# grunwaldlab/krisp

Measured on AMD Instinct MI355X. Metric: k-mers/s sorted+intersected at k=28, higher is better.
Workload: dtype u64

## Files before the change

include/krisp_hip.h:

```cpp
#ifndef KRISP_HIP_H
#define KRISP_HIP_H

#include <stddef.h>
#include <stdint.h>

#ifdef __cplusplus
extern "C" {
#endif

typedef struct kr_ctx kr_ctx;

typedef struct { uint64_t prefix, in_mask, out_mask; } kr_cand;

typedef struct { uint64_t key; uint32_t genome; uint32_t count; } kr_record;

enum {
    KR_OK = 0,
    KR_ERR_HIP = -1,
    KR_ERR_PARAM = -2,
    KR_ERR_CAPACITY = -3,
    KR_ERR_STATE = -4,
    KR_ERR_KEY = -5,
    KR_ERR_HOST = -6
};
// ... 208 lines not shown

int64_t kr_render_records(const kr_record* recs, size_t n, int L, int D, int R, const uint32_t* label_of,
                          size_t n_genomes, const char* const* label_text, size_t n_labels, const uint8_t* label_in,
                          int dot, char** csv, size_t* csv_len, char** align, size_t* align_len);
int64_t kr_render_windows(const uint8_t* rows, size_t n, int L, int D, int R, const uint32_t* cand, const uint32_t* genome,
                          const uint32_t* label_of, size_t n_genomes, const char* const* label_text, size_t n_labels,
                          const uint8_t* label_in, int dot, int rna, char** csv, size_t* csv_len, char** align,
                          size_t* align_len);
void    kr_text_free(void* p);

enum { KR_OPT_SLICE_BASES = 1,
       KR_OPT_GENERIC_INTERSECT = 2,
       KR_OPT_ISECT_FORMAT = 3,
       KR_OPT_ABLATE = 4,
       KR_OPT_WIDE_SLOTS = 5,
       KR_OPT_PLACE_TRIES = 7,
       KR_OPT_ISECT_KERNEL = 8,
       KR_OPT_LANES = 9,
       KR_OPT_LAZY_ORDER = 10,
       KR_OPT_COARSE_REST = 11,
       KR_OPT_COARSE_POOL = 12,
       KR_OPT_JOIN2 = 13,
       KR_OPT_COARSE_ONE_STRAND = 14,
       KR_OPT_WIDE_ORDERED = 6 };
int     kr_set_option(kr_ctx*, int option, int64_t value);

int     kr_sync(kr_ctx*);
int     kr_timer_begin(kr_ctx*);
double  kr_timer_end_ms(kr_ctx*);
int     kr_stage_enable(kr_ctx*, int on);
int     kr_stage_select(kr_ctx*, unsigned stage_mask);
int     kr_stage_reset(kr_ctx*);
double  kr_stage_ms(kr_ctx*, int stage);
int64_t kr_stage_launches(kr_ctx*, int stage);

int64_t kr_debug_fetch(kr_ctx*, int genome_id, int what, void* out, size_t cap_bytes);
int64_t kr_debug_inversions(kr_ctx*, int genome_id);
double  kr_debug_localsort(kr_ctx*, int genome_id, int reps, int mode);
double  kr_debug_intersect(kr_ctx*, const int* genome_ids, int n, const uint8_t* is_ingroup, int reps, int mode);
double  kr_debug_copy_gbps(kr_ctx*, size_t bytes, int reps);
const char* kr_debug_copy_which(kr_ctx*);
int     kr_build_experiments(void);
int     kr_debug_lazy(kr_ctx*, int64_t* out8);
int     kr_debug_isect(kr_ctx*, int64_t* out8);
int     kr_debug_scan(kr_ctx*, int64_t* out8);
int     kr_debug_place(kr_ctx*, double* out8);
int     kr_debug_coarse_pool(kr_ctx*, double* out8);
int     kr_debug_coarse_strand(kr_ctx*, int64_t* out8);
int     kr_debug_comm(kr_ctx*, int64_t* out8);
int     kr_debug_comm_probe(kr_ctx*, size_t bytes, int reps, double* out3);
int64_t kr_debug_cands_selfexchange(kr_ctx*, int apply_filter);
int     kr_debug_comm_hang(kr_ctx*);
int64_t kr_debug_budget_left(kr_ctx*);
int     kr_debug_budget_set(kr_ctx*, int64_t left);
int     kr_debug_info(kr_ctx*, int64_t* out8);

#ifdef __cplusplus
}
#endif
#endif
```

krisp_amd/_native.py:

```python
import ctypes
import os

import numpy as np

HERE = os.path.dirname(os.path.abspath(__file__))
LIB_PATH = os.environ.get("KRISP_HIP_LIB") or os.path.join(HERE, "libkrisp_hip.so")

CAND = np.dtype([("prefix", "<u8"), ("in_mask", "<u8"), ("out_mask", "<u8")])
RECORD = np.dtype([("key", "<u8"), ("genome", "<u4"), ("count", "<u4")])
WIDE_HIT = np.dtype([("cand", "<u4"), ("genome", "<u4"), ("pos", "<u4"), ("strand", "<u4")])
LOC_HIT = np.dtype([("group", "<u4"), ("strand", "<u4"), ("pos", "<u8")])
NEAR_HIT = np.dtype([("target", "<u4"), ("strand", "u1"), ("mismatches", "u1"), ("flank_mismatches", "u1"), ("pad", "u1"),
                     ("pos", "<u8")])
PRODUCT_SITE = np.dtype([("pos", "<u8"), ("entry", "<u4"), ("mismatches", "u1"), ("end_mismatches", "u1"),
                         ("pad", "<u2")])
PRODUCT_HIT = np.dtype([("pos", "<u8"), ("length", "<u4"), ("pair", "<u4"), ("strand", "u1"), ("left_mm", "u1"),
                        ("right_mm", "u1"), ("left_end_mm", "u1"), ("right_end_mm", "u1"), ("pad", "u1", (3,))])
MULTIPLEX_HIT = np.dtype([("pos", "<u8"), ("length", "<u4"), ("fwd", "<u2"), ("rev", "<u2"), ("fwd_mm", "u1"), ("rev_mm", "u1"),
                          ("fwd_end_mm", "u1"), ("rev_end_mm", "u1"), ("pad", "u1", (4,))])
DESIGN_RECORD = np.dtype([("found", "<u4"), ("product_size", "<u4"), ("pair_penalty", "<u4"), ("left_start", "<u2"),
                          ("left_len", "<u2"), ("right_start", "<u2"), ("right_len", "<u2"), ("left_tm", "<i4"), ("right_tm", "<i4"),
                          ("left_gc", "<u2"), ("right_gc", "<u2"), ("left_penalty", "<u4"), ("right_penalty", "<u4"),
                          ("left_self_any", "<i4"), ("left_self_end", "<i4"), ("right_self_any", "<i4"),
                          ("right_self_end", "<i4"), ("pair_any", "<i4"), ("pair_end", "<i4")])
# ... 3 lines not shown
GUIDE_RECORD = np.dtype([("found", "<u4"), ("strand", "<u4"), ("start", "<u4"), ("min_mismatches", "<u4"),
                         ("sum_mismatches", "<u4"), ("gc", "<u4"), ("candidates", "<u4"), ("pad", "<u4")])
GUIDE_HIT_RAW = np.dtype([("guide", "<u4"), ("strand", "u1"), ("mismatches", "u1"), ("pam", "u1"), ("pad", "u1"), ("pos", "<u8"),
                          ("columns", "<u8")])
ASSAY_HIT_RAW = np.dtype([("pos", "<u8"), ("length", "<u4"), ("pair", "<u4"), ("strand", "u1"), ("left_mm", "u1"), ("right_mm", "u1"),
                          ("left_end_mm", "u1"), ("right_end_mm", "u1"), ("hit_strand", "u1"), ("hit_mismatches", "u1"),
                          ("hit_pam", "u1"), ("hit_pos", "<u8"), ("columns", "<u8"), ("guide", "<u4"), ("hit", "<u4")])
GUIDE_BULGE_HIT_RAW = np.dtype([("guide", "<u4"), ("strand", "u1"), ("mismatches", "u1"), ("pam", "u1"), ("bulge", "i1"),
                                ("pos", "<u8"), ("columns", "<u8"), ("bulge_column", "<u4"), ("length", "<u4")])
WIDE_DICT_LEFT, WIDE_DICT_RIGHT, WIDE_GROUPS, WIDE_HITS, WIDE_COUNTS, WIDE_SLOT_BITS, WIDE_NGROUPS, WIDE_BATCH_USED, WIDE_LOCATED, WIDE_KEYS_LISTED = 0, 1, 2, 3, 4, 5, 6, 7, 8, 9
WIDE_MAX_K = 1024
WIDE_MAX_FLANK = 256
COMM_ID_BYTES = 128

SOFT_MAP, SOFT_OMIT = 0, 1
OPT_SLICE_BASES, OPT_GENERIC_INTERSECT, OPT_ISECT_FORMAT, OPT_ABLATE, OPT_WIDE_SLOTS, OPT_WIDE_ORDERED, OPT_PLACE_TRIES = 1, 2, 3, 4, 5, 6, 7
OPT_ISECT_KERNEL = 8
OPT_LANES = 9
OPT_LAZY_ORDER = 10
OPT_COARSE_REST = 11
OPT_COARSE_POOL = 12
OPT_JOIN2 = 13
OPT_COARSE_ONE_STRAND = 14
ERR_KEY, ERR_HOST = -5, -6
STRANDS_BOTH, STRANDS_FORWARD, STRANDS_CANONICAL = 0, 1, 2
STAGES = ["pack", "hist8", "reduce8", "scatter1", "hist2", "scan2", "scatter2", "chunks", "localsort",
          "fallback", "intersect", "compact", "collect", "merge", "locate"]
STAGE_KERNELS = {"pack": "k_pack", "hist8": "k_hist8 (wide path: k_hist8w, slices: k_hist8k)", "reduce8": "k_reduce8a+k_reduce8b",
                 "scatter1": "k_scatter1p (wide path: k_scatter1w, slices: k_scatter1kp)",
                 "hist2": "k_hist16 (or k_hist2)", "scan2": "k_hist16_off (or k_scan2)", "scatter2": "k_scatter2",
                 "chunks": "k_chunk_table", "localsort": "k_localsort2",
                 "fallback": "k_seg_merge", "intersect": "k_intersect3 (+ k_intersect for oversized items)",
                 "compact": "k_scan+k_publish_reset+k_gather_items",
                 "collect": "k_collect_count+k_tile_sums+k_scan+k_tile_apply+k_publish+k_collect_emit",
                 "merge": "k_cands_flag+k_scan+k_cands_compact", "locate": "k_wide_locate"}

_c = ctypes
_P = _c.c_void_p
SYMBOLS = [
    ("kr_create", _P, [_c.c_int, _c.c_size_t]),
    ("kr_destroy", None, [_P]),
    ("kr_last_error", _c.c_char_p, [_P]),
    ("kr_set_params", _c.c_int, [_P, _c.c_int, _c.c_int, _c.c_int, _c.c_int, _c.c_size_t]),
    ("kr_set_strands", _c.c_int, [_P, _c.c_int]),
    ("kr_genome_upload", _c.c_int, [_P, _c.c_int, _P, _c.c_size_t]),
    ("kr_genome_sort", _c.c_int, [_P, _c.c_int]),
# ... 101 lines not shown
    ("kr_genome_fetch_bases", _c.c_int64, [_P, _c.c_int, _P, _c.c_size_t]),
    ("kr_host_free", None, [_P]),
    ("kr_scan_special", _c.c_int64, [_P, _c.c_size_t, _c.c_int, _c.c_int, _P, _c.c_size_t, _P]),
    ("kr_set_option", _c.c_int, [_P, _c.c_int, _c.c_int64]),
    ("kr_sync", _c.c_int, [_P]),
    ("kr_timer_begin", _c.c_int, [_P]),
    ("kr_timer_end_ms", _c.c_double, [_P]),
    ("kr_stage_enable", _c.c_int, [_P, _c.c_int]),
    ("kr_stage_select", _c.c_int, [_P, _c.c_uint]),
    ("kr_stage_reset", _c.c_int, [_P]),
    ("kr_stage_ms", _c.c_double, [_P, _c.c_int]),
    ("kr_stage_launches", _c.c_int64, [_P, _c.c_int]),
    ("kr_debug_fetch", _c.c_int64, [_P, _c.c_int, _c.c_int, _P, _c.c_size_t]),
    ("kr_debug_inversions", _c.c_int64, [_P, _c.c_int]),
    ("kr_debug_localsort", _c.c_double, [_P, _c.c_int, _c.c_int, _c.c_int]),
    ("kr_debug_intersect", _c.c_double, [_P, _P, _c.c_int, _P, _c.c_int, _c.c_int]),
    ("kr_debug_copy_gbps", _c.c_double, [_P, _c.c_size_t, _c.c_int]),
    ("kr_debug_copy_which", _c.c_char_p, [_P]),
    ("kr_mem_info", _c.c_int, [_P, _P]),
    ("kr_debug_comm", _c.c_int, [_P, _P]),
    ("kr_debug_place", _c.c_int, [_P, _P]),
    ("kr_debug_coarse_pool", _c.c_int, [_P, _P]),
    ("kr_debug_coarse_strand", _c.c_int, [_P, _P]),
    ("kr_debug_comm_probe", _c.c_int, [_P, _c.c_size_t, _c.c_int, _P]),
    ("kr_debug_cands_selfexchange", _c.c_int64, [_P, _c.c_int]),
    ("kr_debug_info", _c.c_int, [_P, _P]),
    ("kr_render_records", _c.c_int64, [_P, _c.c_size_t, _c.c_int, _c.c_int, _c.c_int, _P, _c.c_size_t, _P, _c.c_size_t, _P,
                                       _c.c_int, _P, _P, _P, _P]),
    ("kr_text_free", None, [_P]),
    ("kr_debug_isect", _c.c_int, [_P, _P]),
    ("kr_debug_lazy", _c.c_int, [_P, _P]),
    ("kr_debug_scan", _c.c_int, [_P, _P]),
    ("kr_set_mixed_alphabets", _c.c_int, [_P, _c.c_int]),
    ("kr_build_experiments", _c.c_int, []),
    ("kr_comm_set_timeout", _c.c_int, [_P, _c.c_int]),
    ("kr_debug_comm_hang", _c.c_int, [_P]),
    ("kr_debug_budget_left", _c.c_int64, [_P]),
    ("kr_debug_budget_set", _c.c_int, [_P, _c.c_int64]),
]


class GuideParams(ctypes.Structure):
    _fields_ = [("guide_size", _c.c_int32), ("pam5_len", _c.c_int32), ("pam3_len", _c.c_int32), ("pam5", _c.c_uint8 * 8),
                ("pam3", _c.c_uint8 * 8), ("gc_lo", _c.c_int32), ("gc_hi", _c.c_int32), ("min_mismatches", _c.c_int32)]


# ... 776 lines not shown
    def mem_info(self):
        o = np.zeros(4, dtype=np.int64)
        self._check(self.lib.kr_mem_info(self.ctx, _ptr(o)), "kr_mem_info")
        return dict(avail=int(o[0]), total=int(o[1]), used=int(o[2]), budget=int(o[3]))

    def debug_comm(self):
        o = np.zeros(8, dtype=np.int64)
        self._check(self.lib.kr_debug_comm(self.ctx, _ptr(o)), "kr_debug_comm")
        return dict(syncs=int(o[0]), p2p=int(o[1]), collectives=int(o[2]), exchange_us=int(o[3]), reduces=int(o[4]),
                    message_entries=int(o[5]))

    def debug_place(self):
        o = np.zeros(8, dtype=np.float64)
        self._check(self.lib.kr_debug_place(self.ctx, _ptr(o)), "kr_debug_place")
        return dict(candidates=int(o[0]), taken=int(o[1]), fastest_ms=[round(float(x), 4) for x in o[2:6]],
                    median_ms=round(float(o[6]), 4), slowest_ms=round(float(o[7]), 4))

    def debug_coarse_strand(self):
        o = np.zeros(8, dtype=np.int64)
        self._check(self.lib.kr_debug_coarse_strand(self.ctx, _ptr(o)), "kr_debug_coarse_strand")
        return dict(partitions=int(o[0]), calls=int(o[1]), rounds_forward=int(o[2]), rounds_reverse=int(o[3]),
                    last_forward=int(o[4]), last_reverse=int(o[5]), on=int(o[6]))

    def debug_coarse_pool(self):
        o = np.zeros(8, dtype=np.float64)
        self._check(self.lib.kr_debug_coarse_pool(self.ctx, _ptr(o)), "kr_debug_coarse_pool")
        return dict(total=int(o[0]), free=int(o[1]), held=int(o[2]), partitions=int(o[3]), searches=int(o[4]),
                    held_ms=[round(float(o[5]), 4), round(float(o[6]), 4)], on=int(o[7]))

    def comm_set_timeout(self, seconds):
        self._check(self.lib.kr_comm_set_timeout(self.ctx, int(seconds)), "kr_comm_set_timeout")

    def debug_comm_hang(self):
        return self._check(self.lib.kr_debug_comm_hang(self.ctx), "kr_debug_comm_hang")

    def cands_selfexchange(self, apply_filter=False):
        return self._check(self.lib.kr_debug_cands_selfexchange(self.ctx, 1 if apply_filter else 0), "kr_debug_cands_selfexchange")

    def comm_probe(self, nbytes=64 << 10, reps=50):
        o = np.zeros(3, dtype=np.float64)
        self._check(self.lib.kr_debug_comm_probe(self.ctx, nbytes, reps, _ptr(o)), "kr_debug_comm_probe")
        return dict(allreduce_sync_us=round(float(o[0]), 2), sendrecv_self_sync_us=round(float(o[1]), 2),
                    bcast_sync_us=round(float(o[2]), 2), message_bytes=int(nbytes))

    def copy_which(self):
        return (self.lib.kr_debug_copy_which(self.ctx) or b"").decode()
# ... 10 lines not shown
```

krisp_amd/csrc/h_core.inc:

```
static thread_local std::string g_last_error;

struct DevBuf {
    void* p = nullptr;
    size_t bytes = 0;
};

struct Slice {
    DevBuf keys, off, chunkstart, chunkdesc, ovf;
    u64 nmax = 0;
    u32 nchunks = 0;
    int64_t count = -1;
    int res = -1;
};

struct Genome {
    int id = -1;
    size_t n_bases = 0;
    u64 nwords = 0;
    u64 nmax = 0;
    DevBuf bases, wkeys;
    DevBuf wlcnt;
    bool wlist = false;
    u32 wlcap = 0;
    std::vector<Slice> sl;
    bool uploaded = false, sorted = false, finalized = false;
    bool ordered = false;
    bool coarse = false;
    bool one_strand = false;
    DevBuf ckeys;
    double ckeys_ms = 0;
    hipStream_t ckeys_busy = nullptr;
    hipEvent_t ckeys_ev = nullptr;
    bool ckeys_wait = false;
    int64_t partitions = 0;
    DevBuf hits;
    u32 hitcap = 0;
    bool hits_valid = false;
    bool was_anchor = false;
    int64_t count = -1;
    hipEvent_t up_done = nullptr;
};

struct Lane {
    hipStream_t stream = nullptr;
    hipEvent_t done = nullptr;
    bool pending = false;
    DevBuf codes, bad, partial8, base1, tmpkeys, tp, tiledesc, tilehist, wkeys;
    DevBuf partial16, cursor, h16exc;
    DevBuf pass0, base64;
    DevBuf slt, offa, cura;
    void bufs(std::vector<DevBuf*>& v) {
        v.insert(v.end(), {&codes, &bad, &partial8, &base1, &tmpkeys, &tp, &tiledesc, &tilehist, &wkeys, &pass0, &base64,
                           &partial16, &cursor, &h16exc, &slt, &offa, &cura});
    }
};
#define MAX_LANES 8

struct kr_comm;

struct kr_ctx {
    int device = 0;
    kr_comm* comm = nullptr;
    hipStream_t stream = nullptr;
    hipStream_t copy_stream = nullptr;
    Lane lanes[MAX_LANES];
    int nlanes = 0, next_lane = 0;
    int lanes_ready = 0;
    int64_t sorts_done = 0;
    int place_n = 0, place_taken = 0;
    double place_ms[6] = {0, 0, 0, 0, 0, 0};
    size_t place_bytes = 0;
    u64 ex_cap = 0;
    char copy_which[160] = {0};
    u64 lane_maxcount = 0;
    int last_lane = 0;
    int sb = 0, nslices = 1;
    size_t budget = 0, used = 0;
    bool have_params = false;
    Geom g{};
    size_t max_bases = 0;
    std::map<int, Genome> genomes;
    int ls_grid = 768;
    int place_tries = 8;
    bool place_tries_set = false;
    bool shared_gpu = false;
    DevBuf candP;
    DevBuf candA, candB, chunkcnt, chunkpos, flags, blockcnt, blockpos, other, records, nrec, fbdesc, fbsegs;
    DevBuf coltab, collo, colcnt, colpos, coltsum, coltpos, colfirst, colfm;
    int64_t ncand = -1;
    int64_t nrecords = 0;
// ... 454 lines not shown
        c->pool.push_back(p.a);
        c->pool.push_back(p.b);
    }
    c->pending.clear();
}

#define LANES_AUTO 3
#define LANES_AFTER 16
static inline int lanes_used(const kr_ctx* c) {
    if (c->wide.on) return c->wide.lanes > 0 ? c->wide.lanes : (c->nlanes > 1 ? 2 : 1);
    if (c->g.wmode) return 1;
    if (c->nslices > 1) return c->nlanes == 1 || (c->nlanes == 0 && c->sorts_done < 2) ? 1 : 2;
    return c->nlanes > 0 ? c->nlanes : (c->sorts_done >= LANES_AFTER ? LANES_AUTO : 1);
}

static int join_lanes(kr_ctx* c) {
    for (int i = 1; i < MAX_LANES; i++) {
        Lane& ln = c->lanes[i];
        if (!ln.pending) continue;
        HIPCHK(c, hipEventRecord(ln.done, ln.stream));
        HIPCHK(c, hipStreamWaitEvent(c->stream, ln.done, 0));
        ln.pending = false;
    }
    return KR_OK;
}

static int lane_open(kr_ctx* c, Lane& ln) {
    if (ln.stream) return KR_OK;
    HIPCHK(c, hipStreamCreate(&ln.stream));
    HIPCHK(c, hipEventCreateWithFlags(&ln.done, hipEventDisableTiming));
    return KR_OK;
}
static void release_lanes(kr_ctx* c, int first) {
    std::vector<DevBuf*> lb;
    for (int i = first; i < MAX_LANES; i++) c->lanes[i].bufs(lb);
    for (DevBuf* b : lb) release(c, *b);
}
static int ensure_h16exc(kr_ctx* c, Lane& ln, hipStream_t st) {
    if (ln.h16exc.p) return KR_OK;
    int rc;
    if ((rc = ensure(c, ln.h16exc, (1 + 3 * (size_t)H16_EXC_CAP) * 4))) return rc;
    HIPCHK(c, hipMemsetAsync(ln.h16exc.p, 0, 16, st));
    return KR_OK;
}

static void launch_excl_scan(hipStream_t st, const u32* in, u32 n, u32* tsum, u32* tpos, u32* out) {
// ... 31 lines not shown
        c->isect_fmt = e2 ? (atoi(e2) == 1 ? 1 : (atoi(e2) == 2 ? 2 : 0)) : 0;
        const char* e3 = getenv("KR_SLICE_BASES");
        c->opt_slice_bases = e3 ? std::max(0, std::min(4, atoi(e3))) : -1;
        const char* e16 = getenv("KR_FUSE_ANCHOR");
        c->fuse_anchor = e16 ? atoi(e16) != 0 : 1;
        const char* e15 = getenv("KR_LAZY_ORDER");
        c->lazy_order = e15 ? atoi(e15) != 0 : 1;
        const char* e17 = getenv("KR_COARSE_REST");
        c->coarse_rest = e17 ? atoi(e17) != 0 : 1;
        const char* e21 = getenv("KR_COARSE_POOL");
        c->coarse_pool = e21 ? atoi(e21) != 0 : 1;
        const char* e26 = getenv("KR_COARSE_ONE_STRAND");
        c->coarse_one = e26 ? atoi(e26) != 0 : 1;
        const char* e22 = getenv("KR_PLACE_MIN_BYTES");
        if (e22) c->place_min_bytes = (size_t)std::max(0ll, atoll(e22));
        const char* e18 = getenv("KR_COARSE_TCAP");
        if (e18) c->co_tcap = (u32)std::max(1, std::min((int)CO_TCAP, atoi(e18)));
        const char* e19 = getenv("KR_COARSE_HITCAP");
        if (e19) c->co_hitcap = (u32)std::max(1, atoi(e19));
        const char* e20 = getenv("KR_COARSE_GRID");
        if (e20) c->co_grid = (u32)std::max(0, std::min(65536, atoi(e20)));
        const char* e24 = getenv("KR_JOIN2");
        c->join2 = e24 ? atoi(e24) != 0 : 1;
        const char* e25 = getenv("KR_JOIN2_GRID");
        if (e25) c->j2_grid = (u32)std::max(0, std::min(65536, atoi(e25)));
        const char* e23 = getenv("KR_SCAN_GRID");
        if (e23) c->scan_cap = (u32)std::max(0, std::min(65536, atoi(e23)));
        const char* e13 = getenv("KR_SLICE_ROUTE");
        c->slice_route = e13 ? atoi(e13) != 0 : 1;
        const char* e8 = getenv("KR_PLACE_TRIES");
        c->place_tries = e8 ? std::max(1, std::min(16, atoi(e8))) : 8;
        c->place_tries_set = e8 != nullptr;
        const char* e4 = getenv("KR_WIDE_SLOTS");
        c->wide.use_slots = e4 ? atoi(e4) != 0 : true;
        const char* e7 = getenv("KR_WIDE_SHARE");
        c->wide.use_share = e7 ? atoi(e7) != 0 : true;
        const char* e11 = getenv("KR_WIDE_SPECTRUM");
        c->wide.packed_spectrum = e11 ? atoi(e11) != 0 : true;
        const char* e5 = getenv("KR_WIDE_ORDERED");
        c->wide.ordered = e5 ? atoi(e5) != 0 : false;
        int ncu = 256, per = 3;
        (void)hipDeviceGetAttribute(&ncu, hipDeviceAttributeMultiprocessorCount, device);
        if (hipOccupancyMaxActiveBlocksPerMultiprocessor(&per, k_localsort2, LS_THREADS, 0) != hipSuccess || per < 1)
            per = 2;
        c->ls_grid = ncu * per;
        c->ncu = ncu;
// ... 154 lines not shown
        return KR_OK;
    case KR_OPT_GENERIC_INTERSECT:
        c->dbg = (c->dbg & ~32) | (value ? 32 : 0);
        return KR_OK;
    case KR_OPT_ISECT_FORMAT:
        if (value < 0 || value > 2) return fail(c, KR_ERR_PARAM, "KR_OPT_ISECT_FORMAT: 0, 1 or 2");
        c->isect_fmt = (int)value;
        return KR_OK;
    case KR_OPT_ISECT_KERNEL:
        if (value < 0 || value > 2) return fail(c, KR_ERR_PARAM, "KR_OPT_ISECT_KERNEL: 0, 1 or 2");
        c->isect_kernel = (int)value;
        return KR_OK;
    case KR_OPT_WIDE_SLOTS:
        if (value != 0 && value != 1) return fail(c, KR_ERR_PARAM, "KR_OPT_WIDE_SLOTS: 0 or 1");
        c->wide.use_slots = value != 0;
        return KR_OK;
    case KR_OPT_LANES:
        if (value < 0 || value > MAX_LANES) return fail(c, KR_ERR_PARAM, "KR_OPT_LANES: 0 (automatic), 1 .. %d", MAX_LANES);
        HIPCHK(c, hipSetDevice(c->device));
        { int rcj = join_lanes(c); if (rcj) return rcj; }
        HIPCHK(c, hipDeviceSynchronize());
        c->nlanes = (int)value;
        c->next_lane = 0;
        return (c->have_params && c->lane_maxcount) ? ensure_lanes(c, c->lane_maxcount) : KR_OK;
    case KR_OPT_PLACE_TRIES:
        if (value < 1 || value > 16) return fail(c, KR_ERR_PARAM, "KR_OPT_PLACE_TRIES: 1 .. 16");
        c->place_tries = (int)value;
        c->place_tries_set = true;
        return KR_OK;
    case KR_OPT_WIDE_ORDERED:
        if (value != 0 && value != 1) return fail(c, KR_ERR_PARAM, "KR_OPT_WIDE_ORDERED: 0 or 1");
        c->wide.ordered = value != 0;
        return KR_OK;
    case KR_OPT_LAZY_ORDER:
        if (value != 0 && value != 1) return fail(c, KR_ERR_PARAM, "KR_OPT_LAZY_ORDER: 0 or 1");
        c->lazy_order = (int)value;
        return KR_OK;
    case KR_OPT_COARSE_REST:
        if (value != 0 && value != 1) return fail(c, KR_ERR_PARAM, "KR_OPT_COARSE_REST: 0 or 1");
        c->coarse_rest = (int)value;
        return KR_OK;
    case KR_OPT_COARSE_POOL:
        if (value != 0 && value != 1) return fail(c, KR_ERR_PARAM, "KR_OPT_COARSE_POOL: 0 or 1");
        c->coarse_pool = (int)value;
        return KR_OK;
    case KR_OPT_COARSE_ONE_STRAND:
        if (value != 0 && value != 1) return fail(c, KR_ERR_PARAM, "KR_OPT_COARSE_ONE_STRAND: 0 or 1");
        c->coarse_one = (int)value;
        return KR_OK;
    case KR_OPT_JOIN2:
        if (value != 0 && value != 1) return fail(c, KR_ERR_PARAM, "KR_OPT_JOIN2: 0 or 1");
        c->join2 = (int)value;
        return KR_OK;
    case KR_OPT_ABLATE:
#ifdef KR_ABLATE
        c->dbg = (c->dbg & 32) | ((int)value & ~32);
        return KR_OK;
#else
        return fail(c, KR_ERR_PARAM, "KR_OPT_ABLATE needs a -DKR_ABLATE build");
#endif
    default:
        return fail(c, KR_ERR_PARAM, "unknown option %d", option);
    }
}

int kr_set_strands(kr_ctx* c, int mode) {
    if (!c || !c->have_params) return fail(c, KR_ERR_STATE, "kr_set_params first");
    if (mode < KR_STRANDS_BOTH || mode > KR_STRANDS_CANONICAL) return fail(c, KR_ERR_PARAM, "unknown strand mode %d", mode);
    if (c->wide.on && mode == KR_STRANDS_CANONICAL) return fail(c, KR_ERR_PARAM, "the wide path emits both strands or the forward one");
    if (!c->genomes.empty()) return fail(c, KR_ERR_STATE, "kr_set_strands after genomes were uploaded");
    c->g.strands = mode;
    c->wide.strands = mode;
    return KR_OK;
}

int kr_set_allow(kr_ctx* c, unsigned base_mask) {
// ... 305 lines not shown
        const auto kw = g.wmode == 1 ? k_scatter1w<1> : g.wcmode == 2 ? k_scatter1w<3> : k_scatter1w<2>;
        hipLaunchKernelGGL(kw, dim3(NWG), dim3(P1_T), 0, st, codes, bad, nwords, base1, base64, rowoff, dst, g);
    } else {
        const auto kp = fast ? (big ? k_scatter1p<0, 1, 1> : k_scatter1p<0, 0, 1>)
                             : g.strands ? (big ? k_scatter1p<2, 1> : k_scatter1p<2, 0>) : (big ? k_scatter1p<0, 1> : k_scatter1p<0, 0>);
        hipLaunchKernelGGL(kp, dim3(NWG), dim3(P1_T), 0, st, codes, bad, nwords, base1, base64, rowoff, dst, dst_keys, g);
    }
}

static void launch_scatter2(hipStream_t st, const u64* src, u64* dst, const uint2* tiledesc, u32 ntmax,
                            const u32* tilehist, u32* cursor, int b, int shl = 0, u32 region_n = 0) {
    hipLaunchKernelGGL(k_scatter2<2 * P2_T>, dim3(ntmax), dim3(2 * P2_T), 0, st, src, dst, tiledesc, tilehist, cursor, b, shl, region_n);
}

static void launch_hist8(kr_ctx* c, Genome& G, Lane& ln, hipStream_t st, const Geom& g, bool one = false) {
    const auto kh = one ? k_hist8<3> : g.wmode == 1 ? k_hist8w<1> : g.wmode ? (g.wcmode == 2 ? k_hist8w<3> : k_hist8w<2>) : g.strands ? k_hist8<2> : k_hist8<0>;
    hipLaunchKernelGGL(kh, dim3(NWG), dim3(P1_T), 0, st, (const u64*)ln.codes.p, (const u32*)ln.bad.p, G.nwords,
                       (u32*)ln.partial8.p, g);
}

static constexpr u32 P2_KEYS = 2 * P2_TILE;
static u32 p2_tiles(u64 nmax) { return (u32)(nmax / P2_KEYS) + 257; }

static Lane& peek_lane(kr_ctx* c) {
    if (c->next_lane >= lanes_used(c)) c->next_lane = 0;
    return c->lanes[c->next_lane];
}

static Geom pass0_geom(const kr_ctx* c, bool counting = false) {
    Geom g0 = c->g;
    g0.sbits = 0;
    g0.slice = 0;
    if (counting && g0.wmode == 2 && g0.wcache) g0.wcmode = g0.wlcnt ? 3 : 1;
    return g0;
}

static int count_slices(kr_ctx* c, Genome& G) {
    int rc;
    if ((rc = ensure_lanes(c, 16))) return rc;
    Lane& ln = peek_lane(c);
    hipStream_t st = ln.stream;
    ln.pending = true;
    if (G.up_done && st != c->stream) HIPCHK(c, hipStreamWaitEvent(st, G.up_done, 0));
    launch_pack(c, G, ln, st);
    reset_slices(c, G);
    std::vector<u32> tot(256);
    u64 maxcount = 0;
    G.nmax = 0;
    genome_unsorted(G);
// ... 140 lines not shown
}
int kr_genome_partition(kr_ctx* c, int id) {
    if (!c) return KR_ERR_PARAM;
    return genome_sort(c, id, false, coarse_eligible(c));
}

struct SortPlan {
    bool reuse_count;
    bool coarse;
    bool one;
    bool lazy;
    bool sliced, route2, fine16;
    bool cached_keys;
    int cached_mode;
    int nba;
    u32 h16_ranges;
    int nsl, helper;
};

static bool one_strand_form(const kr_ctx* c) {
    return c->coarse_one && c->g.D == 1 && p1_fast_form(c->g) && c->g.L >= 5 && c->g.R < c->g.L && c->g.sbits == 0;
}

static SortPlan sort_plan(const kr_ctx* c, const Genome& G, const Lane& ln, bool reuse_count, bool coarse) {
    SortPlan p{};
    p.reuse_count = reuse_count;
    p.coarse = coarse;
    p.one = coarse && !reuse_count && one_strand_form(c);
    p.cached_keys = reuse_count && c->g.wmode == 2 && c->g.wcache;
    p.cached_mode = c->g.wlcnt ? 4 : 2;
    p.sliced = c->nslices > 1;
    static const bool lazy_wide = [] { const char* e = getenv("KR_LAZY_WIDE"); return e ? atoi(e) != 0 : true; }();
    p.lazy = c->lazy_order && (lazy_wide || (!c->wide.on && c->g.wmode == 0)) && !c->custom_layout && c->g.strands == 0 &&
             !c->order_wanted && !(G.was_anchor && !c->i3_last_ua);
    p.nba = 8 + c->g.sbits;
    p.route2 = p.sliced && USE_HIST16 && c->slice_route && c->g.wmode == 0 && c->g.strands == 0 && 2 * c->g.L >= p.nba && p.nba <= 16;
    p.h16_ranges = H16_RANGES;
    if (p.route2)
        while (p.h16_ranges < NWG && G.nmax / ((u64)p.h16_ranges * 256) > 30000) p.h16_ranges *= 2;
    p.fine16 = USE_HIST16 && c->g.b > 8 && !p.sliced && c->g.wmode == 0 && c->g.strands == 0 && 2 * c->g.L >= c->g.b;
    p.nsl = p.route2 ? slice_lanes(c) : 1;
    p.helper = SLICE_HELPER + SLICE_HELPERS * (int)(&ln - c->lanes);
    return p;
}

static int take_lane(kr_ctx* c, Genome& G, Lane*& taken) {
    if (lanes_used(c) > c->lanes_ready) {
        int rcl = ensure_lanes(c, c->lane_maxcount);
        if (rcl && c->nlanes == 0) {
            release_lanes(c, 1);
            c->nlanes = 1;
            c->lanes_ready = 1;
            c->next_lane = 0;
            c->err.clear();
            rcl = KR_OK;
        }
        if (rcl) return rcl;
    }
    Lane& ln = peek_lane(c);
    c->last_lane = c->next_lane;
    c->next_lane = (c->next_lane + 1) % lanes_used(c);
    ln.pending = true;
    hipStream_t st = ln.stream;
    if (G.up_done && st != c->stream) HIPCHK(c, hipStreamWaitEvent(st, G.up_done, 0));
    taken = &ln;
    return KR_OK;
}

static void coarse_pool_step(kr_ctx* c, Genome& G, bool coarse) {
    const size_t cbytes = ((size_t)c->lane_maxcount + 2) * 8;
    if (G.ckeys.p && (!coarse || !c->coarse_pool || G.ckeys.bytes < cbytes)) coarse_pool_return(c, G);
    if (coarse) {
        G.partitions++;
        if (c->coarse_pool && !G.ckeys.p) (void)coarse_pool_take(c, G, cbytes);
    }
}

static void pass_pack(kr_ctx* c, Genome& G, Lane& ln) {
    StageScope sc(c, KR_ST_PACK, ln.stream);
    launch_pack(c, G, ln, ln.stream);
}

static int pass0(kr_ctx* c, Genome& G, const SortPlan& p, Lane& ln) {
    hipStream_t st = ln.stream;
// ... 181 lines not shown
    hipStream_t ss = ls.stream;
    {
        StageScope sc(c, KR_ST_CHUNKS, ss);
        hipLaunchKernelGGL(k_chunk_table, dim3((S.nchunks + 255) / 256), dim3(256), 0, ss, (const u32*)S.off.p, 1u << c->g.b,
                           S.nchunks, (uint4*)S.chunkdesc.p, (u32*)S.ovf.p, (p.fine16 || p.route2) ? (u32*)ln.h16exc.p : (u32*)nullptr);
    }
    if (p.lazy) {
        c->lazy_skipped++;
        return;
    }
    StageScope sc(c, KR_ST_LOCALSORT, ss);
    launch_localsort(c, S, S.chunkdesc, S.nchunks, ss);
}

static int genome_sort(kr_ctx* c, int id, bool reuse_count, bool coarse) {
    if (!c) return KR_ERR_PARAM;
    auto it = c->genomes.find(id);
    if (it == c->genomes.end() || !it->second.uploaded) return fail(c, KR_ERR_STATE, "genome %d not uploaded", id);
    if (it->second.sl.empty()) return fail(c, KR_ERR_STATE, "genome %d has no slice plan (wide windows: use kr_wide_run)", id);
    HIPCHK(c, hipSetDevice(c->device));
    Genome& G = it->second;
    c->sorts_done++;
    int rc;
    Lane* lane;
    if ((rc = take_lane(c, G, lane))) return rc;
    Lane& ln = *lane;
    genome_unsorted(G);
    coarse_pool_step(c, G, coarse);
    const SortPlan p = sort_plan(c, G, ln, reuse_count, coarse);
    if (p.sliced) {
        if ((rc = pass0(c, G, p, ln))) return rc;
    } else if (!reuse_count) {
        pass_pack(c, G, ln);
    }
    if (p.nsl > 1 && (rc = slice_lanes_start(c, p, ln))) return rc;
    u64 region = 0;
    for (int s = 0; s < c->nslices; s++) {
        Slice& S = G.sl[s];
        Lane& ls = (p.nsl > 1 && s % p.nsl) ? c->lanes[p.helper + s % p.nsl - 1] : ln;
        const u64* src = (const u64*)ln.pass0.p + region;
        region += S.nmax;
        S.count = -1;
        u64* pass1_dst;
        if ((rc = pass1_target(c, G, p, ls, S, pass1_dst))) return rc;
        if (p.route2) pass1_route2(c, p, ln, ls, S, s, src, pass1_dst);
        else pass1_counted(c, G, p, ln, ls, S, s, src, pass1_dst);
        if (coarse) {
            coarse_exit(c, ls, S, p.one);
            continue;
        }
        if ((rc = pass2(c, G, p, ln, ls, S))) return rc;
        chunks_and_order(c, p, ln, ls, S);
// ... 102 lines not shown
    return KR_OK;
}

static int finalize(kr_ctx* c, const std::vector<Genome*>& gs, bool already_synced = false, bool* repaired = nullptr) {
    if (repaired) *repaired = false;
    std::vector<Slice*> todo;
    std::vector<Genome*> tg;
    for (Genome* G : gs)
        if ((G->sorted || G->coarse) && !G->finalized) {
            tg.push_back(G);
            for (Slice& S : G->sl) todo.push_back(&S);
        }
    if (tg.empty()) return KR_OK;
    hipStream_t st = c->stream;
    if (!already_synced) {
        int rcj = join_lanes(c);
        if (rcj) return rcj;
    }
    std::vector<u32> novf(todo.size()), total(todo.size());
    if (!already_synced) {
        for (size_t i0 = 0; i0 < todo.size(); i0 += PUB_CAP) {
            publish_slices(c, todo.data() + i0, std::min<size_t>(PUB_CAP, todo.size() - i0), st);
            HIPCHK(c, hipStreamSynchronize(st));
        }
        HIPCHK(c, hipGetLastError());
    }
    for (size_t i = 0; i < todo.size(); i++) {
        const volatile u32* w = c->mbox + MB_SLICE0 + 2 * todo[i]->res;
        novf[i] = w[0];
        total[i] = w[1];
    }
    for (size_t i = 0; i < todo.size(); i++) {
        Slice& S = *todo[i];
        S.count = total[i];
        if (novf[i]) {
            if (repaired) *repaired = true;
            int rc = repair_slice(c, S, novf[i], total[i], st);
            if (rc) return rc;
        }
    }
    for (Genome* G : tg) {
        G->count = 0;
        for (Slice& S : G->sl) G->count += S.count;
        G->finalized = true;
    }
    return KR_OK;
// ... 164 lines not shown
```

krisp_amd/csrc/h_intersect.inc:

```
static int64_t intersect_once(kr_ctx* c, const int* ids, int n, const uint8_t* is_in, int apply_filter, bool* redo);

static int64_t cands_merge_device(kr_ctx* c, size_t m, int have_other, int apply_filter);

static inline int fmode(const kr_ctx* c, int apply_filter) { return apply_filter ? (c->mixed_alphabets ? 2 : 1) : 0; }

int kr_set_mixed_alphabets(kr_ctx* c, int on) {
    if (!c) return KR_ERR_PARAM;
    c->mixed_alphabets = on != 0;
    return KR_OK;
}

#define KR_MAX_CANDS 0xFFFFFF00ull
static int cands_fit(kr_ctx* c, uint64_t n, const char* who) {
    if (n < KR_MAX_CANDS) return KR_OK;
    return fail(c, KR_ERR_CAPACITY, "%s: a candidate list of %llu entries exceeds the %llu a list may hold (an intersection that "
                "nothing prunes: give both ingroup and outgroup genomes to one call, or fewer genomes per call)", who,
                (unsigned long long)n, (unsigned long long)KR_MAX_CANDS);
}

static int cands_compact_room(kr_ctx* c, u32 n) {
    const size_t nblk = ((size_t)n + 255) / 256;
    int rc;
    if ((rc = ensure(c, c->flags, (size_t)n * 4))) return rc;
    if ((rc = ensure(c, c->blockcnt, (nblk + 2) * 4))) return rc;
// ... 108 lines not shown
            HIPCHK(c, hipMemsetAsync(cnt, 0, CS_CLS * 4, st));
            hipLaunchKernelGGL(k_strand_count, dim3(cgrid), dim3(CS_T), 0, st, (const kr_cand*)c->candB.p, nC, S, cnt);
            hipLaunchKernelGGL(k_strand_tables, dim3(1), dim3(CS_CLS), 0, st, (const u32*)cnt, ca, c->co_tcap, cls, cursor, ust, rows,
                               c->mbox + 56);
            hipLaunchKernelGGL(k_strand_fill, dim3(cgrid), dim3(CS_T), 0, st, (const kr_cand*)c->candB.p, nC, S, cursor, ents);
            hipLaunchKernelGGL(k_coarse_probe<1>, dim3(grid), dim3(CO_T), 0, st, ca, (const u32*)cls, (const u32*)ust, (const u32*)rows,
                               (const kr_cand*)c->candB.p, (u32*)c->co_state.p, c->co_tcap, g.pmask, g.LRrel, (const CoEnt*)ents, S);
        } else {
            hipLaunchKernelGGL(k_coarse_tables, dim3(1), dim3(256), 0, st, (const kr_cand*)c->candB.p, nC, ca, c->co_tcap, cb, ust, rows);
            hipLaunchKernelGGL(k_coarse_probe<0>, dim3(grid), dim3(CO_T), 0, st, ca, (const u32*)cb, (const u32*)ust, (const u32*)rows,
                               (const kr_cand*)c->candB.p, (u32*)c->co_state.p, c->co_tcap, g.pmask, g.LRrel, (const CoEnt*)nullptr,
                               CoStrand{});
        }
    }
    for (Genome* G : cg)
        if (G->ckeys.p) G->ckeys_busy = st;
    {
        StageScope sc(c, KR_ST_MERGE, st);
        hipLaunchKernelGGL(k_coarse_flag, dim3(nblk), dim3(256), 0, st, (kr_cand*)c->candB.p, nC, (const u32*)c->co_state.p, need,
                           fmode(c, 1), (u32*)c->flags.p, (u32*)c->blockcnt.p);
        cands_compact_enqueue(c, nC, st, true);
        hipLaunchKernelGGL(k_coarse_publish, dim3(1), dim3(64), 0, st, pub, c->mbox + 32);
    }
    HIPCHK(c, hipStreamSynchronize(st));
    HIPCHK(c, hipGetLastError());
    for (Genome* G : cg) G->ckeys_busy = nullptr;
    if (one) {
        c->one_calls++;
        for (int q = 0; q < 2; q++) {
            c->one_last[q] = ((volatile u32*)c->mbox)[56 + q];
            c->one_rounds[q] += c->one_last[q];
        }
    }
    for (size_t j = 0; j < cg.size(); j++)
        if (((volatile u32*)c->mbox)[32 + j] > hitcap) {
            c->ncand = -1;
            return KR_COARSE_PASS;
        }
    const u32 total = ((volatile u32*)c->mbox)[16];
    cands_compact_adopt(c, total);
    for (Genome* G : cg) G->hits_valid = true;
    c->coarse_done += (int64_t)cg.size();
    {
        int want = 0;
        for (Genome* G : cg) want += !G->ckeys.p && G->partitions >= 2;
        if (want > 0) coarse_pool_grow(c, want);
    }
    return total;
// ... 522 lines not shown
    a.gid = (const u32*)((uint64_t*)c->coltab.p + 2 * np);
    a.n = n;
    a.nslices = c->nslices;
    a.ibo = nullptr;
    a.arena = nullptr;
    a.mcnt = nullptr;
    const Geom g = slice_geom(c, 0);
    if (arena_on) {
        const size_t npairs = (size_t)nc * (size_t)n;
        if ((rc = ensure(c, c->touchdesc, npairs * COL_CAPM * 8 + npairs * 4 + 64))) return rc;
        if ((rc = ensure(c, c->touchovf, 64))) return rc;
        u64* arena = (u64*)c->touchdesc.p;
        u32* mcnt = (u32*)(arena + npairs * COL_CAPM);
        HIPCHK(c, hipMemsetAsync(c->touchovf.p, 0, 16, st));
        a.ibo = (const u32*)((uint64_t*)c->coltab.p + 2 * np + (n + 1) / 2);
        a.arena = arena;
        a.mcnt = mcnt;
        StageScope sc(c, KR_ST_COLLECT);
        if (any_coarse) HIPCHK(c, hipMemsetAsync(mcnt, 0, npairs * 4, st));
        if (touch)
            hipLaunchKernelGGL(k_collect_scan, dim3((u32)((npairs + 3) / 4)), dim3(256), 0, st, (const kr_cand*)c->candB.p, (u32)npairs, a, g,
                               arena, mcnt, (u32*)c->touchovf.p);
        if (any_coarse) {
            for (int i = 0; i < n; i++)
                if (gs[i]->coarse)
                    hipLaunchKernelGGL(k_coarse_rows, dim3(1024), dim3(256), 0, st, (const u32*)gs[i]->hits.p, gs[i]->hitcap,
                                       (const kr_cand*)c->candB.p, nc, (u32)n, (u32)i, g.pmask, arena, mcnt);
            hipLaunchKernelGGL(k_coarse_rowsort, dim3((u32)((npairs + 255) / 256)), dim3(256), 0, st, (u32)npairs, (u32)n, a.ibo, arena,
                               mcnt, (u32*)c->touchovf.p);
        }
        hipLaunchKernelGGL(k_publish, dim3(1), dim3(64), 0, st, (const u32*)c->touchovf.p, (const u32*)nullptr,
                           (const u32*)nullptr, c->mbox + 20);
        if (touch) c->lazy_touch++;
    }
    u64 done = 0;
    for (u32 c0 = 0; c0 < nc; c0 += per) {
        const u32 cc = std::min(per, nc - c0), np2 = cc * (u32)n;
        const kr_cand* cand = (const kr_cand*)c->candB.p + c0;
        CollectArgs ac = a;
        if (arena_on) {
            ac.arena = a.arena + (size_t)c0 * n * COL_CAPM;
            ac.mcnt = a.mcnt + (size_t)c0 * n;
        }
        const u32 ntiles = (np2 + 2047) / 2048;
        u32 total = 0;
        {
            StageScope sc(c, KR_ST_COLLECT);
            hipLaunchKernelGGL(k_collect_count, dim3((np2 + 255) / 256), dim3(256), 0, st, cand, np2, ac, g,
                               (u32*)c->collo.p, (u32*)c->colcnt.p, (u64*)c->colfirst.p, (u32*)c->colfm.p);
            hipLaunchKernelGGL(k_tile_sums, dim3(ntiles), dim3(256), 0, st, (const u32*)c->colcnt.p, np2, (u32*)c->coltsum.p);
// ... 51 lines not shown
```

krisp_amd/csrc/h_misc.inc:

```
double kr_debug_localsort(kr_ctx* c, int id, int reps, int mode) {
    if (!c || mode != 0) return -1.0;
    auto it = c->genomes.find(id);
    if (it != c->genomes.end() && ensure_fine(c, it->second)) return -1.0;
    if (it == c->genomes.end() || !it->second.sorted || it->second.sl.empty()) return -1.0;
    if (ensure_ordered(c, {&it->second}) || finalize(c, {&it->second})) return -1.0;
    Slice& S = it->second.sl[0];
    hipStream_t st = c->stream;
    const u32 grid = std::min<u32>(S.nchunks, (u32)c->ls_grid);
    auto launch = [&]() {
        hipLaunchKernelGGL(k_localsort2, dim3(grid), dim3(LS_THREADS), 0, st, (u64*)S.keys.p, (const u32*)S.off.p,
                           (const uint4*)S.chunkdesc.p, S.nchunks, c->g.b, (u32*)S.ovf.p,
                           (uint4*)((char*)S.ovf.p + 16));
    };
    hipEvent_t a, b;
    (void)hipEventCreate(&a);
    (void)hipEventCreate(&b);
    launch();
    (void)hipEventRecord(a, st);
    for (int r = 0; r < reps; r++) launch();
    (void)hipEventRecord(b, st);
    (void)hipEventSynchronize(b);
    float ms = 0;
    (void)hipEventElapsedTime(&ms, a, b);
    (void)hipEventDestroy(a);
// ... 237 lines not shown
    out8[1] = (double)c->cpool_free.size();
    out8[2] = held;
    out8[3] = (double)c->cpool_partitions;
    out8[4] = (double)c->cpool_searches;
    out8[5] = lo;
    out8[6] = hi;
    out8[7] = c->coarse_pool;
    return KR_OK;
}

int kr_debug_coarse_strand(kr_ctx* c, int64_t* o) {
    if (!c || !o) return KR_ERR_PARAM;
    o[0] = c->one_partitions;
    o[1] = c->one_calls;
    o[2] = c->one_rounds[0];
    o[3] = c->one_rounds[1];
    o[4] = c->one_last[0];
    o[5] = c->one_last[1];
    o[6] = c->coarse_one;
    o[7] = 0;
    return KR_OK;
}

int kr_debug_isect(kr_ctx* c, int64_t* o) {
    if (!c || !o) return KR_ERR_PARAM;
    o[0] = c->isect_ovf_items;
    o[1] = c->isect_refall;
    o[2] = c->i3_last_T;
    o[3] = c->i3_last_mlog;
    o[4] = c->i3_last_tags;
    o[5] = lanes_used(c);
    o[6] = c->j2_launches;
    o[7] = c->j2_full;
    return KR_OK;
}

int kr_debug_scan(kr_ctx* c, int64_t* o) {
    if (!c || !o) return KR_ERR_PARAM;
    o[0] = c->scan_dbg[0];
    o[1] = c->scan_dbg[1];
    o[2] = c->scan_cap;
    o[3] = c->scan_dbg[2];
    o[4] = o[5] = o[6] = o[7] = 0;
    return KR_OK;
}

// ... 52 lines not shown
```

krisp_amd/csrc/k_coarse.inc:

```

#include "co_units.inc"

#define CO_T 1024
#define CO_SLOT_LOG 13
#define CO_SLOTS (1u << CO_SLOT_LOG)
#define CO_BM_LOG 17
#define CO_QCAP 2048
#define CO_TCAP 6144
#define CO_EMPTY 0xFFFFFFFFu
#define CO_UNROLL 4
#define CO_ITER (2u * CO_T * CO_UNROLL)
#define CO_HB 1024
#define CO_MAXG 24
#define CO_ROW (2 * CO_MAXG)

struct CoarseArgs {
    const u64* keys[CO_MAXG];
    const u32* off[CO_MAXG];
    u32* hits[CO_MAXG];
    u32 hitcap[CO_MAXG];
    u32 bit[CO_MAXG];
    u32 side[CO_MAXG];
    u32 n;
};
// ... 367 lines not shown
    bool keep = false;
    if (i < n) {
        const u32 st = state[i];
        keep = (st & need) == need;
        if (keep) {
            kr_cand c = cur[i];
            c.in_mask |= st & 15u;
            c.out_mask |= (st >> 4) & 15u;
            keep = passes_filter(c.in_mask, c.out_mask, 1, mode);
            if (keep) cur[i] = c;
        }
        flags[i] = keep ? 1u : 0u;
    }
    u32 tot;
    block_compact(keep, waves, tot);
    if (threadIdx.x == 0) blockcnt[blockIdx.x] = tot;
}

struct CoarsePub { const u32* cnt[CO_MAXG]; int n; };
__global__ void k_coarse_publish(CoarsePub p, u32* __restrict__ host) {
    if (blockIdx.x == 0 && (int)threadIdx.x < p.n) host[threadIdx.x] = *p.cnt[threadIdx.x];
}

__global__ __launch_bounds__(256) void k_coarse_rows(const u32* __restrict__ hits, u32 hitcap, const kr_cand* __restrict__ cands,
                                                     u32 nc, u32 n, u32 gi, u64 pmask, u64* __restrict__ arena,
                                                     u32* __restrict__ mcnt) {
    const u32 nh = min(hits[0], hitcap);
    const u64* __restrict__ hk = (const u64*)(hits + 4);
    for (u32 i = blockIdx.x * blockDim.x + threadIdx.x; i < nh; i += gridDim.x * blockDim.x) {
        const u64 key = hk[i], pre = key & pmask;
        u32 l = 0, r = nc;
        while (l < r) {
            const u32 mid = l + ((r - l) >> 1);
            if (cands[mid].prefix < pre) l = mid + 1; else r = mid;
        }
        if (l < nc && cands[l].prefix == pre) {
            const u32 row = l * n + gi;
            const u32 at = atomicAdd(&mcnt[row], 1u);
            if (at < COL_CAPM) arena[(u64)row * COL_CAPM + at] = key;
        }
    }
}

__global__ __launch_bounds__(256) void k_coarse_rowsort(u32 npairs, u32 n, const u32* __restrict__ ibo, u64* __restrict__ arena,
                                                        u32* __restrict__ mcnt, u32* __restrict__ overflow) {
    const u32 idx = blockIdx.x * blockDim.x + threadIdx.x;
    if (idx >= npairs || ibo[idx % n] != 2u) return;
    const u32 m = mcnt[idx];
    if (m > COL_CAPM) {
// ... 20 lines not shown
```

Baseline: 131.5 billion.

## Assign sort lanes by estimated load and batch coarse row kernels

```diff
diff --git a/include/krisp_hip.h b/include/krisp_hip.h
--- a/include/krisp_hip.h
+++ b/include/krisp_hip.h
@@ -254,6 +254,7 @@
        KR_OPT_COARSE_POOL = 12,
        KR_OPT_JOIN2 = 13,
        KR_OPT_COARSE_ONE_STRAND = 14,
+       KR_OPT_LANE_PICK = 15,
        KR_OPT_WIDE_ORDERED = 6 };
 int     kr_set_option(kr_ctx*, int option, int64_t value);
 
@@ -279,6 +280,7 @@
 int     kr_debug_place(kr_ctx*, double* out8);
 int     kr_debug_coarse_pool(kr_ctx*, double* out8);
 int     kr_debug_coarse_strand(kr_ctx*, int64_t* out8);
+int     kr_debug_lanes(kr_ctx*, int64_t* out20);
 int     kr_debug_comm(kr_ctx*, int64_t* out8);
 int     kr_debug_comm_probe(kr_ctx*, size_t bytes, int reps, double* out3);
 int64_t kr_debug_cands_selfexchange(kr_ctx*, int apply_filter);
diff --git a/krisp_amd/_native.py b/krisp_amd/_native.py
--- a/krisp_amd/_native.py
+++ b/krisp_amd/_native.py
@@ -49,6 +49,7 @@
 OPT_COARSE_POOL = 12
 OPT_JOIN2 = 13
 OPT_COARSE_ONE_STRAND = 14
+OPT_LANE_PICK = 15
 ERR_KEY, ERR_HOST = -5, -6
 STRANDS_BOTH, STRANDS_FORWARD, STRANDS_CANONICAL = 0, 1, 2
 STAGES = ["pack", "hist8", "reduce8", "scatter1", "hist2", "scan2", "scatter2", "chunks", "localsort",
@@ -196,6 +197,7 @@
     ("kr_debug_place", _c.c_int, [_P, _P]),
     ("kr_debug_coarse_pool", _c.c_int, [_P, _P]),
     ("kr_debug_coarse_strand", _c.c_int, [_P, _P]),
+    ("kr_debug_lanes", _c.c_int, [_P, _P]),
     ("kr_debug_comm_probe", _c.c_int, [_P, _c.c_size_t, _c.c_int, _P]),
     ("kr_debug_cands_selfexchange", _c.c_int64, [_P, _c.c_int]),
     ("kr_debug_info", _c.c_int, [_P, _P]),
@@ -1018,6 +1020,12 @@
         return dict(partitions=int(o[0]), calls=int(o[1]), rounds_forward=int(o[2]), rounds_reverse=int(o[3]),
                     last_forward=int(o[4]), last_reverse=int(o[5]), on=int(o[6]))
 
+    def debug_lanes(self):
+        o = np.zeros(20, dtype=np.int64)
+        self._check(self.lib.kr_debug_lanes(self.ctx, _ptr(o)), "kr_debug_lanes")
+        return dict(lanes=int(o[0]), pick=int(o[1]), moved=int(o[2]), finalize_waits=int(o[3]),
+                    taken=[int(x) for x in o[4:20:2]], load=[int(x) for x in o[5:20:2]])
+
     def debug_coarse_pool(self):
         o = np.zeros(8, dtype=np.float64)
         self._check(self.lib.kr_debug_coarse_pool(self.ctx, _ptr(o)), "kr_debug_coarse_pool")
diff --git a/krisp_amd/csrc/h_core.inc b/krisp_amd/csrc/h_core.inc
--- a/krisp_amd/csrc/h_core.inc
+++ b/krisp_amd/csrc/h_core.inc
@@ -1,4 +1,6 @@
 static thread_local std::string g_last_error;
+
+#include "lane_pick.inc"
 
 struct DevBuf {
     void* p = nullptr;
@@ -45,6 +47,8 @@
     hipStream_t stream = nullptr;
     hipEvent_t done = nullptr;
     bool pending = false;
+    u64 load = 0;
+    int64_t taken = 0;
     DevBuf codes, bad, partial8, base1, tmpkeys, tp, tiledesc, tilehist, wkeys;
     DevBuf partial16, cursor, h16exc;
     DevBuf pass0, base64;
@@ -66,6 +70,9 @@
     Lane lanes[MAX_LANES];
     int nlanes = 0, next_lane = 0;
     int lanes_ready = 0;
+    int lane_pick = 1;
+    int64_t lane_moved = 0;
+    int64_t finalize_waits = 0;
     int64_t sorts_done = 0;
     int place_n = 0, place_taken = 0;
     double place_ms[6] = {0, 0, 0, 0, 0, 0};
@@ -566,6 +573,7 @@
         HIPCHK(c, hipStreamWaitEvent(c->stream, ln.done, 0));
         ln.pending = false;
     }
+    for (int i = 0; i < MAX_LANES; i++) c->lanes[i].load = 0;
     return KR_OK;
 }
 
@@ -643,6 +651,8 @@
         if (e20) c->co_grid = (u32)std::max(0, std::min(65536, atoi(e20)));
         const char* e24 = getenv("KR_JOIN2");
         c->join2 = e24 ? atoi(e24) != 0 : 1;
+        const char* e27 = getenv("KR_LANE_PICK");
+        c->lane_pick = e27 ? atoi(e27) != 0 : 1;
         const char* e25 = getenv("KR_JOIN2_GRID");
         if (e25) c->j2_grid = (u32)std::max(0, std::min(65536, atoi(e25)));
         const char* e23 = getenv("KR_SCAN_GRID");
@@ -843,6 +853,7 @@
         HIPCHK(c, hipDeviceSynchronize());
         c->nlanes = (int)value;
         c->next_lane = 0;
+        for (int i = 0; i < MAX_LANES; i++) c->lanes[i].load = 0;
         return (c->have_params && c->lane_maxcount) ? ensure_lanes(c, c->lane_maxcount) : KR_OK;
     case KR_OPT_PLACE_TRIES:
         if (value < 1 || value > 16) return fail(c, KR_ERR_PARAM, "KR_OPT_PLACE_TRIES: 1 .. 16");
@@ -873,6 +884,10 @@
         if (value != 0 && value != 1) return fail(c, KR_ERR_PARAM, "KR_OPT_JOIN2: 0 or 1");
         c->join2 = (int)value;
         return KR_OK;
+    case KR_OPT_LANE_PICK:
+        if (value != 0 && value != 1) return fail(c, KR_ERR_PARAM, "KR_OPT_LANE_PICK: 0 or 1");
+        c->lane_pick = (int)value;
+        return KR_OK;
     case KR_OPT_ABLATE:
 #ifdef KR_ABLATE
         c->dbg = (c->dbg & 32) | ((int)value & ~32);
@@ -1224,9 +1239,15 @@
 static constexpr u32 P2_KEYS = 2 * P2_TILE;
 static u32 p2_tiles(u64 nmax) { return (u32)(nmax / P2_KEYS) + 257; }
 
+static bool lane_pick_on(const kr_ctx* c) { return c->lane_pick && !c->wide.on && c->g.wmode == 0 && c->nslices == 1; }
+
 static Lane& peek_lane(kr_ctx* c) {
-    if (c->next_lane >= lanes_used(c)) c->next_lane = 0;
-    return c->lanes[c->next_lane];
+    static_assert(MAX_LANES == LP_MAX_LANES, "lane_pick.inc counts the same lanes");
+    const int lanes = lanes_used(c);
+    if (c->next_lane >= lanes) c->next_lane = 0;
+    uint64_t load[MAX_LANES];
+    for (int i = 0; i < MAX_LANES; i++) load[i] = c->lanes[i].load;
+    return c->lanes[lp_pick(load, lanes, c->next_lane, lane_pick_on(c))];
 }
 
 static Geom pass0_geom(const kr_ctx* c, bool counting = false) {
@@ -1413,7 +1434,7 @@
     return c->coarse_one && c->g.D == 1 && p1_fast_form(c->g) && c->g.L >= 5 && c->g.R < c->g.L && c->g.sbits == 0;
 }
 
-static SortPlan sort_plan(const kr_ctx* c, const Genome& G, const Lane& ln, bool reuse_count, bool coarse) {
+static SortPlan sort_plan(const kr_ctx* c, const Genome& G, bool reuse_count, bool coarse) {
     SortPlan p{};
     p.reuse_count = reuse_count;
     p.coarse = coarse;
@@ -1431,11 +1452,11 @@
         while (p.h16_ranges < NWG && G.nmax / ((u64)p.h16_ranges * 256) > 30000) p.h16_ranges *= 2;
     p.fine16 = USE_HIST16 && c->g.b > 8 && !p.sliced && c->g.wmode == 0 && c->g.strands == 0 && 2 * c->g.L >= c->g.b;
     p.nsl = p.route2 ? slice_lanes(c) : 1;
-    p.helper = SLICE_HELPER + SLICE_HELPERS * (int)(&ln - c->lanes);
+    p.helper = SLICE_HELPER;
     return p;
 }
 
-static int take_lane(kr_ctx* c, Genome& G, Lane*& taken) {
+static int take_lane(kr_ctx* c, Genome& G, int kind, Lane*& taken) {
     if (lanes_used(c) > c->lanes_ready) {
         int rcl = ensure_lanes(c, c->lane_maxcount);
         if (rcl && c->nlanes == 0) {
@@ -1443,14 +1464,19 @@
             c->nlanes = 1;
             c->lanes_ready = 1;
             c->next_lane = 0;
+            for (int i = 0; i < MAX_LANES; i++) c->lanes[i].load = 0;
             c->err.clear();
             rcl = KR_OK;
         }
         if (rcl) return rcl;
     }
     Lane& ln = peek_lane(c);
-    c->last_lane = c->next_lane;
-    c->next_lane = (c->next_lane + 1) % lanes_used(c);
+    const int at = (int)(&ln - c->lanes);
+    c->lane_moved += at != c->next_lane;
+    c->last_lane = at;
+    c->next_lane = (at + 1) % lanes_used(c);
+    ln.load += lp_cost(kind, G.nmax);
+    ln.taken++;
     ln.pending = true;
     hipStream_t st = ln.stream;
     if (G.up_done && st != c->stream) HIPCHK(c, hipStreamWaitEvent(st, G.up_done, 0));
@@ -1678,12 +1704,15 @@
     Genome& G = it->second;
     c->sorts_done++;
     int rc;
+    SortPlan p = sort_plan(c, G, reuse_count, coarse);
+    const int kind = p.coarse ? (p.one ? LP_COARSE_ONE : LP_COARSE_TWO) : (p.lazy ? LP_FINE_LAZY : LP_FINE_ORDERED);
     Lane* lane;
-    if ((rc = take_lane(c, G, lane))) return rc;
+    if ((rc = take_lane(c, G, kind, lane))) return rc;
     Lane& ln = *lane;
+    p.nsl = p.route2 ? slice_lanes(c) : 1;
+    p.helper = SLICE_HELPER + SLICE_HELPERS * (int)(&ln - c->lanes);
     genome_unsorted(G);
     coarse_pool_step(c, G, coarse);
-    const SortPlan p = sort_plan(c, G, ln, reuse_count, coarse);
     if (p.sliced) {
         if ((rc = pass0(c, G, p, ln))) return rc;
     } else if (!reuse_count) {
@@ -1832,6 +1861,7 @@
         for (size_t i0 = 0; i0 < todo.size(); i0 += PUB_CAP) {
             publish_slices(c, todo.data() + i0, std::min<size_t>(PUB_CAP, todo.size() - i0), st);
             HIPCHK(c, hipStreamSynchronize(st));
+            c->finalize_waits++;
         }
         HIPCHK(c, hipGetLastError());
     }
diff --git a/krisp_amd/csrc/h_intersect.inc b/krisp_amd/csrc/h_intersect.inc
--- a/krisp_amd/csrc/h_intersect.inc
+++ b/krisp_amd/csrc/h_intersect.inc
@@ -154,8 +154,20 @@
         cands_compact_enqueue(c, nC, st, true);
         hipLaunchKernelGGL(k_coarse_publish, dim3(1), dim3(64), 0, st, pub, c->mbox + 32);
     }
+    std::vector<Genome*> open_coarse;
+    {
+        std::vector<Slice*> open_slices;
+        for (Genome* G : cg)
+            if (!G->finalized) {
+                open_coarse.push_back(G);
+                for (Slice& S : G->sl) open_slices.push_back(&S);
+            }
+        if (open_slices.size() > PUB_CAP) open_coarse.clear();
+        else publish_slices(c, open_slices.data(), open_slices.size(), st);
+    }
     HIPCHK(c, hipStreamSynchronize(st));
     HIPCHK(c, hipGetLastError());
+    if ((rc = finalize(c, open_coarse, true))) return rc;
     for (Genome* G : cg) G->ckeys_busy = nullptr;
     if (one) {
         c->one_calls++;
@@ -724,10 +736,17 @@
             hipLaunchKernelGGL(k_collect_scan, dim3((u32)((npairs + 3) / 4)), dim3(256), 0, st, (const kr_cand*)c->candB.p, (u32)npairs, a, g,
                                arena, mcnt, (u32*)c->touchovf.p);
         if (any_coarse) {
-            for (int i = 0; i < n; i++)
-                if (gs[i]->coarse)
-                    hipLaunchKernelGGL(k_coarse_rows, dim3(1024), dim3(256), 0, st, (const u32*)gs[i]->hits.p, gs[i]->hitcap,
-                                       (const kr_cand*)c->candB.p, nc, (u32)n, (u32)i, g.pmask, arena, mcnt);
+            CoarseRows cr{};
+            u32 ncr = 0;
+            for (int i = 0; i < n; i++) {
+                if (!gs[i]->coarse) continue;
+                if (ncr == CO_MAXG) return fail(c, KR_ERR_STATE, "kr_collect: more than %d coarse genomes", CO_MAXG);
+                cr.hits[ncr] = (const u32*)gs[i]->hits.p;
+                cr.hitcap[ncr] = gs[i]->hitcap;
+                cr.gi[ncr++] = (u32)i;
+            }
+            hipLaunchKernelGGL(k_coarse_rows, dim3(1024, ncr), dim3(256), 0, st, cr, (const kr_cand*)c->candB.p, nc,
+                               (u32)n, g.pmask, arena, mcnt);
             hipLaunchKernelGGL(k_coarse_rowsort, dim3((u32)((npairs + 255) / 256)), dim3(256), 0, st, (u32)npairs, (u32)n, a.ibo, arena,
                                mcnt, (u32*)c->touchovf.p);
         }
diff --git a/krisp_amd/csrc/h_misc.inc b/krisp_amd/csrc/h_misc.inc
--- a/krisp_amd/csrc/h_misc.inc
+++ b/krisp_amd/csrc/h_misc.inc
@@ -283,6 +283,19 @@
     return KR_OK;
 }
 
+int kr_debug_lanes(kr_ctx* c, int64_t* o) {
+    if (!c || !o) return KR_ERR_PARAM;
+    o[0] = lanes_used(c);
+    o[1] = c->lane_pick;
+    o[2] = c->lane_moved;
+    o[3] = c->finalize_waits;
+    for (int l = 0; l < MAX_LANES; l++) {
+        o[4 + 2 * l] = c->lanes[l].taken;
+        o[5 + 2 * l] = (int64_t)c->lanes[l].load;
+    }
+    return KR_OK;
+}
+
 int kr_debug_isect(kr_ctx* c, int64_t* o) {
     if (!c || !o) return KR_ERR_PARAM;
     o[0] = c->isect_ovf_items;
diff --git a/krisp_amd/csrc/k_coarse.inc b/krisp_amd/csrc/k_coarse.inc
--- a/krisp_amd/csrc/k_coarse.inc
+++ b/krisp_amd/csrc/k_coarse.inc
@@ -413,9 +413,15 @@
     if (blockIdx.x == 0 && (int)threadIdx.x < p.n) host[threadIdx.x] = *p.cnt[threadIdx.x];
 }
 
-__global__ __launch_bounds__(256) void k_coarse_rows(const u32* __restrict__ hits, u32 hitcap, const kr_cand* __restrict__ cands,
-                                                     u32 nc, u32 n, u32 gi, u64 pmask, u64* __restrict__ arena,
-                                                     u32* __restrict__ mcnt) {
+struct CoarseRows {
+    const u32* hits[CO_MAXG];
+    u32 hitcap[CO_MAXG];
+    u32 gi[CO_MAXG];
+};
+__global__ __launch_bounds__(256) void k_coarse_rows(CoarseRows r, const kr_cand* __restrict__ cands, u32 nc, u32 n, u64 pmask,
+                                                     u64* __restrict__ arena, u32* __restrict__ mcnt) {
+    const u32* __restrict__ hits = r.hits[blockIdx.y];
+    const u32 hitcap = r.hitcap[blockIdx.y], gi = r.gi[blockIdx.y];
     const u32 nh = min(hits[0], hitcap);
     const u64* __restrict__ hk = (const u64*)(hits + 4);
     for (u32 i = blockIdx.x * blockDim.x + threadIdx.x; i < nh; i += gridDim.x * blockDim.x) {
diff --git a/krisp_amd/csrc/lane_pick.inc b/krisp_amd/csrc/lane_pick.inc
--- /dev/null
+++ b/krisp_amd/csrc/lane_pick.inc
@@ -0,0 +1,40 @@
+#include <stdint.h>
+
+#define LP_MAX_LANES 8
+
+enum LpKind { LP_COARSE_ONE = 0, LP_COARSE_TWO = 1, LP_FINE_LAZY = 2, LP_FINE_ORDERED = 3 };
+
+static inline uint64_t lp_weight(int kind) {
+    switch (kind) {
+    case LP_COARSE_ONE: return 180;
+    case LP_COARSE_TWO: return 305;
+    case LP_FINE_LAZY: return 790;
+    default: return 1150;
+    }
+}
+
+static inline uint64_t lp_cost(int kind, uint64_t nmax) {
+    const uint64_t cap = (uint64_t)1 << 40;
+    return lp_weight(kind) * (nmax < cap ? nmax : cap);
+}
+
+static inline int lp_pick(const uint64_t* load, int lanes, int next, int on) {
+    if (!on) return next;
+    int best = next;
+    for (int k = 1; k < lanes; k++) {
+        const int l = (next + k) % lanes;
+        if (load[l] < load[best]) best = l;
+    }
+    return best;
+}
+
+static inline int lp_take(uint64_t* load, int lanes, int* next, int on, uint64_t cost) {
+    const int l = lp_pick(load, lanes, *next, on);
+    load[l] += cost;
+    *next = (l + 1) % lanes;
+    return l;
+}
+
+static inline void lp_join(uint64_t* load) {
+    for (int l = 0; l < LP_MAX_LANES; l++) load[l] = 0;
+}
```

New measurement: 131.4 billion. No clear change (-0.0%).
